# microsoft/Spartan2

Measured on AMD Instinct MI355X. Metric: sha256_spartan prove(): R1CS constraints/sec (prove wall-clock in ms_per_step), higher is better.
Workload: dtype u256 modular integer (8 x u32 Montgomery limbs; T256 scalar/base fields)

## Files before the change

spartan2_amd/csrc/capi_sparse.hip:

```cpp
#include <algorithm>
#include <cstring>
#include <string>
#include <vector>

#include "core.hpp"
#include "device_utils.hpp"
#include "kernels_sat.hpp"

using sp::fail;
typedef FqP S;

namespace spk {

struct SplitDev {
  const unsigned* sptr;
  const unsigned* sidx;
  const signed char* scode;
  const unsigned* gptr;
  const unsigned* gidx;
  const fe_t* gval;
};

__device__ __forceinline__ fe_t small_mul(int code, const fe_t& x) {
  const int a = code < 0 ? -code : code;
  fe_t r;
  switch (a) {
    case 1: r = x; break;
    case 2: r = fe_dbl<S>(x); break;
    case 3: r = fe_add<S>(fe_dbl<S>(x), x); break;
    case 4: r = fe_dbl<S>(fe_dbl<S>(x)); break;
// ... 77 lines not shown
    while (pending) {
      const int owner = __ffsll((long long)pending) - 1;
      pending &= pending - 1;
      const size_t r = wbase + (size_t)owner;
      const fe_t part = wave_sum(gather_major(m, r, z, lane, 64));
      if ((int)lane == owner) acc = part;
    }
    if (valid) {
      if (base) acc = fe_add<S>(acc, base[row]);
      out[row] = acc;
    }
  }
}

__global__ void __launch_bounds__(256) k_round0_products(const fe_t* __restrict__ A, const fe_t* __restrict__ B, const fe_t* __restrict__ C, size_t half,
                                                         fe_t* __restrict__ p0, fe_t* __restrict__ p1) {
  for (size_t i = (size_t)blockIdx.x * blockDim.x + threadIdx.x; i < half; i += (size_t)gridDim.x * blockDim.x) {
    const fe_t a0 = A[i], a1 = A[i + half], b0 = B[i], b1 = B[i + half], c0 = C[i];
    p0[i] = fe_sub<S>(fe_mul<S>(a0, b0), c0);
    p1[i] = fe_mul<S>(fe_sub<S>(a1, a0), fe_sub<S>(b1, b0));
  }
}

struct PolyAbcArgs {
  SplitDev m[3];
  fe_t r, r2;
};
constexpr unsigned LONG_COLUMN = 512;
__device__ __forceinline__ unsigned col_len(const PolyAbcArgs& a, size_t col) {
  unsigned n = 0;
#pragma unroll
  for (int i = 0; i < 3; ++i) n += (a.m[i].sptr[col + 1] - a.m[i].sptr[col]) + (a.m[i].gptr[col + 1] - a.m[i].gptr[col]);
  return n;
}
constexpr unsigned LONG_NB_MAX = 128;
__device__ __forceinline__ unsigned long_nb(unsigned len) {
  unsigned nb = (len + 2047) / 2048;
  return nb < 1 ? 1 : (nb > LONG_NB_MAX ? LONG_NB_MAX : nb);
}
__global__ void __launch_bounds__(256) k_polyabc_short_and_long(PolyAbcArgs a, const fe_t* __restrict__ rx, const unsigned* __restrict__ order, size_t n_short,
                                                                fe_t* __restrict__ out, const unsigned* __restrict__ long_cols, unsigned n_long,
                                                                fe_t* __restrict__ partials, unsigned* __restrict__ tickets, unsigned short_blocks,
                                                                size_t zero_from, size_t zero_n, int permuted) {
  __shared__ fe_t smem[3 * 4];
  __shared__ unsigned s_last;
  const unsigned long_blocks = LONG_NB_MAX * n_long;
  if (blockIdx.x >= long_blocks + short_blocks) {
    uint4* z = reinterpret_cast<uint4*>(out + zero_from);
    const size_t n16 = zero_n * 2, nb = gridDim.x - long_blocks - short_blocks;
    for (size_t i = (size_t)(blockIdx.x - long_blocks - short_blocks) * blockDim.x + threadIdx.x; i < n16; i += nb * blockDim.x) z[i] = make_uint4(0u, 0u, 0u, 0u);
    return;
  }
  if (blockIdx.x < long_blocks) {
    const unsigned by = blockIdx.x / LONG_NB_MAX, bx = blockIdx.x % LONG_NB_MAX;
    const size_t col = long_cols[by];
    const size_t at = permuted ? n_short + by : col;
    const unsigned nb = long_nb(col_len(a, at));
    if (bx >= nb) return;
    fe_t acc[3];
#pragma unroll
    for (int i = 0; i < 3; ++i) acc[i] = gather_major(a.m[i], at, rx, bx * blockDim.x + threadIdx.x, nb * blockDim.x);
    block_sum<3>(acc, smem);
    fe_t* trip = partials + ((size_t)by * LONG_NB_MAX) * 3;
    if (threadIdx.x == 0) {
      unsigned* dst = reinterpret_cast<unsigned*>(trip + (size_t)bx * 3);
#pragma unroll
      for (int i = 0; i < 3; ++i)
#pragma unroll
        for (int w = 0; w < 8; ++w) __hip_atomic_store(dst + 8 * i + w, acc[i].v[w], __ATOMIC_RELAXED, __HIP_MEMORY_SCOPE_AGENT);
      s_last = __hip_atomic_fetch_add(tickets + by, 1u, __ATOMIC_ACQ_REL, __HIP_MEMORY_SCOPE_AGENT) == nb - 1 ? 1u : 0u;
    }
    __syncthreads();
    if (!s_last) return;
#pragma unroll
    for (int i = 0; i < 3; ++i) {
      acc[i] = fe_zero();
      if (threadIdx.x < nb) {
        const unsigned* src = reinterpret_cast<const unsigned*>(trip + (size_t)threadIdx.x * 3 + i);
#pragma unroll
        for (int w = 0; w < 8; ++w) acc[i].v[w] = __hip_atomic_load(src + w, __ATOMIC_RELAXED, __HIP_MEMORY_SCOPE_AGENT);
      }
    }
    __syncthreads();
    block_sum<3>(acc, smem);
    if (threadIdx.x == 0) {
      __hip_atomic_store(tickets + by, 0u, __ATOMIC_RELAXED, __HIP_MEMORY_SCOPE_AGENT);
      out[col] = fe_add<S>(fe_add<S>(acc[0], fe_mul<S>(a.r, acc[1])), fe_mul<S>(a.r2, acc[2]));
    }
    return;
  }
  const size_t nblk = short_blocks;
  for (size_t i = (size_t)(blockIdx.x - long_blocks) * blockDim.x + threadIdx.x; i < n_short; i += nblk * blockDim.x) {
    const size_t col = order[i], at = permuted ? i : col;
    fe_t sa = gather_major_x4(a.m[0], at, rx), sb = gather_major_x4(a.m[1], at, rx), sc = gather_major_x4(a.m[2], at, rx);
    if (!fe_is_zero(sb)) sa = fe_add<S>(sa, fe_mul<S>(a.r, sb));
    if (!fe_is_zero(sc)) sa = fe_add<S>(sa, fe_mul<S>(a.r2, sc));
    out[col] = sa;
  }
}
}

#include "kernels_mateval.hpp"
#include "kernels_polyabc_batch.hpp"
#include "kernels_spmv_multi.hpp"
#include "kernels_nifs_layers.hpp"

namespace {

struct SplitHost {
  std::vector<unsigned> sptr, sidx, gptr, gidx;
  std::vector<signed char> scode;
  std::vector<fe_t> gval;
};
struct SplitOnDevice {
  unsigned *sptr = nullptr, *sidx = nullptr, *gptr = nullptr, *gidx = nullptr;
  signed char* scode = nullptr;
  fe_t* gval = nullptr;
  unsigned max_len = 0;
  spk::SplitDev view() const { return spk::SplitDev{sptr, sidx, scode, gptr, gidx, gval}; }
  void release() {
// ... 25 lines not shown

template <class T>
int upload(T** dst, const std::vector<T>& src) {
  size_t bytes = (src.empty() ? 1 : src.size()) * sizeof(T);
  hipError_t e = hipMalloc((void**)dst, bytes);
  if (e != hipSuccess) return fail(SP_ERR_NO_DEVICE, std::string("hipMalloc: ") + hipGetErrorString(e));
  if (!src.empty()) e = hipMemcpy(*dst, src.data(), src.size() * sizeof(T), hipMemcpyHostToDevice);
  if (e != hipSuccess) return fail(SP_ERR_NO_DEVICE, std::string("hipMemcpy: ") + hipGetErrorString(e));
  return SP_OK;
}
int upload_split(const SplitHost& h, SplitOnDevice* d) {
  int rc;
  if ((rc = upload(&d->sptr, h.sptr))) return rc;
  if ((rc = upload(&d->sidx, h.sidx))) return rc;
  if ((rc = upload(&d->scode, h.scode))) return rc;
  if ((rc = upload(&d->gptr, h.gptr))) return rc;
  if ((rc = upload(&d->gidx, h.gidx))) return rc;
  d->max_len = 0;
  for (size_t i = 0; i + 1 < h.sptr.size(); ++i) {
    const unsigned l = (h.sptr[i + 1] - h.sptr[i]) + (h.gptr[i + 1] - h.gptr[i]);
    if (l > d->max_len) d->max_len = l;
  }
  return upload(&d->gval, h.gval);
}

struct Entry {
  unsigned major, minor;
  int code;
  fe_t val;
};
SplitHost build_split(size_t n_major, const std::vector<Entry>& es) {
  SplitHost h;
  h.sptr.assign(n_major + 1, 0);
  h.gptr.assign(n_major + 1, 0);
  for (const Entry& e : es) (e.code ? h.sptr : h.gptr)[e.major + 1]++;
  for (size_t i = 0; i < n_major; ++i) {
    h.sptr[i + 1] += h.sptr[i];
    h.gptr[i + 1] += h.gptr[i];
  }
  h.sidx.resize(h.sptr[n_major]);
  h.scode.resize(h.sptr[n_major]);
  h.gidx.resize(h.gptr[n_major]);
  h.gval.resize(h.gptr[n_major]);
  std::vector<unsigned> sc(h.sptr.begin(), h.sptr.end() - 1), gc(h.gptr.begin(), h.gptr.end() - 1);
  for (const Entry& e : es) {
    if (e.code) {
      unsigned p = sc[e.major]++;
      h.sidx[p] = e.minor;
      h.scode[p] = (signed char)e.code;
    } else {
      unsigned p = gc[e.major]++;
      h.gidx[p] = e.minor;
      h.gval[p] = e.val;
    }
  }
  return h;
}

}

struct sp_shape {
  sp_dims dims;
  size_t num_vars = 0, num_cols = 0;
  SplitOnDevice row[3];
  SplitOnDevice filtered[3];
  SplitOnDevice col[3];
  unsigned* d_long_cols = nullptr;
  unsigned* d_short_order = nullptr;
  size_t n_short = 0;
  size_t n_long_cols = 0;
  bool col_permuted = false;
  uint64_t nnz[3] = {0, 0, 0}, nnz_filtered[3] = {0, 0, 0};
};

extern "C" {

int sp_shape_from_csr(sp_ctx* c, const sp_csr* A, const sp_csr* Bm, const sp_csr* C, const sp_dims* dims, sp_shape** out) {
  (void)c;
  sp_shape* s = new sp_shape();
  s->dims = *dims;
  s->num_vars = dims->num_shared + dims->num_precommitted + dims->num_rest;
  s->num_cols = s->num_vars + 1 + dims->num_public + dims->num_challenges;
  const size_t nrows = dims->num_cons, col_min = dims->num_shared + dims->num_precommitted, nr_used = dims->num_cons_unpadded;
  const sp_csr* M[3] = {A, Bm, C};
  Classifier cls;
  std::vector<unsigned> col_count(s->num_cols, 0);
  std::vector<SplitHost> col_host(3);
  for (int m = 0; m < 3; ++m) {
    const size_t nnz = M[m]->indptr[nrows];
    s->nnz[m] = nnz;
    std::vector<Entry> all, filt, bycol;
    all.reserve(nnz);
    for (size_t r = 0; r < nrows; ++r) {
      for (uint64_t k = M[m]->indptr[r]; k < M[m]->indptr[r + 1]; ++k) {
        Entry e;
        e.major = (unsigned)r;
        e.minor = M[m]->indices[k];
        if (e.minor >= s->num_cols) {
          delete s;
          return fail(SP_ERR_INVALID_INPUT_LENGTH, "sp_shape_from_csr: column index out of range");
        }
        memcpy(&e.val, M[m]->data + 4 * k, 32);
        e.code = cls.code(e.val);
        all.push_back(e);
        if (r < nr_used && e.minor >= col_min) filt.push_back(e);
      }
    }
    s->nnz_filtered[m] = filt.size();
    std::vector<unsigned> cptr(s->num_cols + 1, 0);
    for (const Entry& e : all)
      if (e.major < nr_used) cptr[e.minor + 1]++;
    for (size_t i = 0; i < s->num_cols; ++i) cptr[i + 1] += cptr[i];
    bycol.resize(cptr[s->num_cols]);
    {
      std::vector<unsigned> cur(cptr.begin(), cptr.end() - 1);
      for (const Entry& e : all)
        if (e.major < nr_used) {
          Entry t = e;
          t.major = e.minor;
          t.minor = e.major;
          bycol[cur[e.minor]++] = t;
        }
    }
    for (size_t i = 0; i < s->num_cols; ++i) col_count[i] += cptr[i + 1] - cptr[i];
    int rc;
    col_host[m] = build_split(s->num_cols, bycol);
    if ((rc = upload_split(build_split(nrows, all), &s->row[m])) || (rc = upload_split(build_split(nrows, filt), &s->filtered[m]))) {
      delete s;
      return rc;
    }
  }
  std::vector<unsigned> long_cols;
  for (size_t i = 0; i < s->num_cols; ++i)
    if (col_count[i] >= spk::LONG_COLUMN) long_cols.push_back((unsigned)i);
  s->n_long_cols = long_cols.size();
  int rc = upload(&s->d_long_cols, long_cols);
  if (rc) {
    sp_shape_free(s);
    return rc;
  }
  {
    std::vector<unsigned> order;
    order.reserve(s->num_cols);
    for (size_t i = 0; i < s->num_cols; ++i)
      if (col_count[i] < spk::LONG_COLUMN) order.push_back((unsigned)i);
    auto cnt6 = [&](unsigned col, unsigned out6[6]) {
      for (int m = 0; m < 3; ++m) {
        out6[2 * m] = col_host[m].sptr[col + 1] - col_host[m].sptr[col];
        out6[2 * m + 1] = col_host[m].gptr[col + 1] - col_host[m].gptr[col];
      }
    };
    auto by_len = [&](unsigned x, unsigned y) {
      if (col_count[x] != col_count[y]) return col_count[x] > col_count[y];
      unsigned a[6], b[6];
      cnt6(x, a);
      cnt6(y, b);
      for (int k = 0; k < 5; ++k)
        if (a[k] != b[k]) return a[k] > b[k];
      return false;
    };
    static const int order_mode = [] {
      const char* e = getenv("SPARTAN_POLYABC_ORDER");
      return !e ? 0 : (e[0] == 'n' ? 1 : (e[0] == 'w' ? 2 : 0));
    }();
    if (order_mode == 0) std::stable_sort(order.begin(), order.end(), by_len);
    else if (order_mode == 2)
    {
      const char* w = getenv("SPARTAN_POLYABC_WINDOW");
      const size_t win = w && atol(w) > 0 ? (size_t)atol(w) : 4096;
      for (size_t lo = 0; lo < order.size(); lo += win) std::stable_sort(order.begin() + lo, order.begin() + std::min(order.size(), lo + win), by_len);
    }
    s->n_short = order.size();
    if ((rc = upload(&s->d_short_order, order))) {
      sp_shape_free(s);
      return rc;
    }
    static const bool permuted = [] {
      const char* e = getenv("SPARTAN_POLYABC_LAYOUT");
      return !(e && e[0] == 'n');
    }();
    s->col_permuted = permuted;
    std::vector<unsigned> seq;
    if (permuted) {
      seq = order;
      seq.insert(seq.end(), long_cols.begin(), long_cols.end());
    }
    for (int m = 0; m < 3; ++m) {
      if (!permuted) {
        if ((rc = upload_split(col_host[m], &s->col[m]))) {
          sp_shape_free(s);
          return rc;
        }
        continue;
      }
      const SplitHost& h = col_host[m];
      SplitHost q;
      q.sptr.assign(seq.size() + 1, 0);
      q.gptr.assign(seq.size() + 1, 0);
      q.sidx.reserve(h.sidx.size());
      q.scode.reserve(h.scode.size());
      q.gidx.reserve(h.gidx.size());
      q.gval.reserve(h.gval.size());
      for (size_t pos = 0; pos < seq.size(); ++pos) {
        const unsigned col = seq[pos];
        q.sidx.insert(q.sidx.end(), h.sidx.begin() + h.sptr[col], h.sidx.begin() + h.sptr[col + 1]);
        q.scode.insert(q.scode.end(), h.scode.begin() + h.sptr[col], h.scode.begin() + h.sptr[col + 1]);
        q.gidx.insert(q.gidx.end(), h.gidx.begin() + h.gptr[col], h.gidx.begin() + h.gptr[col + 1]);
        q.gval.insert(q.gval.end(), h.gval.begin() + h.gptr[col], h.gval.begin() + h.gptr[col + 1]);
        q.sptr[pos + 1] = (unsigned)q.sidx.size();
        q.gptr[pos + 1] = (unsigned)q.gidx.size();
      }
      if ((rc = upload_split(q, &s->col[m]))) {
        sp_shape_free(s);
        return rc;
      }
    }
  }
  SP_HIP(hipDeviceSynchronize());
  *out = s;
  return SP_OK;
}
void sp_shape_free(sp_shape* s) {
  if (!s) return;
  for (int m = 0; m < 3; ++m) {
    s->row[m].release();
    s->filtered[m].release();
    s->col[m].release();
  }
  hipFree(s->d_long_cols);
  hipFree(s->d_short_order);
  delete s;
}

int sp_shape_info(const sp_shape* s, uint64_t out[8]) {
  if (!s || !out) return fail(SP_ERR_INVALID_INPUT_LENGTH, "sp_shape_info: null argument");
  for (int m = 0; m < 3; ++m) {
    out[m] = s->nnz[m];
    out[3 + m] = s->nnz_filtered[m];
  }
  out[6] = s->n_long_cols;
  out[7] = s->n_short;
  return SP_OK;
}

static int spmv3(sp_ctx* c, const sp_shape* s, const SplitOnDevice* mats, const uint64_t* nnz, const sp_table* z, const sp_table* const* base,
                 sp_table** outs, const char* what) {
  const size_t nrows = s->dims.num_cons;
  if (z->len != s->num_cols) return fail(SP_ERR_INVALID_WITNESS_LENGTH, "multiply_vec: z has the wrong length");
  spk::Spmv3Args a;
  for (int m = 0; m < 3; ++m) {
    if (outs[m]->cap < nrows) return fail(SP_ERR_INVALID_INPUT_LENGTH, "multiply_vec: output table too short");
// ... 68 lines not shown
  const sp_table* base[3] = {caz, cbz, ccz};
  return spmv3(c, s, s->filtered, s->nnz_filtered, z, base, outs, "spmv_incremental");
}

int sp_multiply_vec_incremental_round0(sp_ctx* c, const sp_shape* s, const sp_table* z, const sp_table* caz, const sp_table* cbz, const sp_table* ccz, sp_table* az,
                                       sp_table* bz, sp_table* cz, sp_table* p0, sp_table* p1) {
  const size_t nrows = s->dims.num_cons, half = nrows / 2;
  if (nrows < 2) return fail(SP_ERR_INVALID_INPUT_LENGTH, "multiply_vec_incremental_round0: needs at least two rows");
  if (p0->cap < half || p1->cap < half) return fail(SP_ERR_INVALID_INPUT_LENGTH, "multiply_vec_incremental_round0: product tables too short");
  int rc = sp_multiply_vec_incremental(c, s, z, caz, cbz, ccz, az, bz, cz);
  if (rc) return rc;
  p0->len = p1->len = half;
  p0->lo_eff = p0->hi_eff = p1->lo_eff = p1->hi_eff = (size_t)-1;
  size_t blocks = (half + 255) / 256;
  if (blocks > 8192) blocks = 8192;
  c->timed("round0_products", 224ull * half, [&] { hipLaunchKernelGGL(spk::k_round0_products, dim3((unsigned)blocks), dim3(256), 0, c->stream, az->d, bz->d, cz->d, half, p0->d, p1->d); });
  return SP_OK;
}

int sp_poly_abc(sp_ctx* c, const sp_shape* s, const sp_table* rx, const uint64_t r_[4], size_t out_len, sp_table* out) {
  if (rx->len != s->dims.num_cons) return fail(SP_ERR_INVALID_INPUT_LENGTH, "poly_ABC: rx must have num_cons elements");
  if (out_len < s->num_cols || out->cap < out_len) return fail(SP_ERR_INVALID_INPUT_LENGTH, "poly_ABC: output too short");
  spk::PolyAbcArgs a;
  for (int m = 0; m < 3; ++m) a.m[m] = s->col[m].view();
  memcpy(&a.r, r_, 32);
  a.r2 = fe_mul<S>(a.r, a.r);
  const size_t ticket_bytes = (s->n_long_cols + 1) * sizeof(unsigned);
  const bool fresh = c->ws_bytes[sp_ctx::WS_POLYABC_TICKETS] < ticket_bytes;
  fe_t* partials = (fe_t*)c->workspace(sp_ctx::WS_POLYABC_PARTIALS, (s->n_long_cols + 1) * spk::LONG_NB_MAX * 3 * sizeof(fe_t));
  unsigned* tickets = (unsigned*)c->workspace(sp_ctx::WS_POLYABC_TICKETS, ticket_bytes);
  if (!partials || !tickets) return SP_ERR_NO_DEVICE;
  if (fresh) SP_HIP(hipMemsetAsync(tickets, 0, c->ws_bytes[sp_ctx::WS_POLYABC_TICKETS], c->stream));
  size_t blocks = (s->n_short + 255) / 256;
  if (blocks > 4096) blocks = 4096;
  if (blocks == 0) blocks = 1;
  const uint64_t bytes = 36ull * (s->nnz[0] + s->nnz[1] + s->nnz[2]) + 32ull * out_len;
  const size_t zero_n = out_len - s->num_cols;
  size_t zblocks = (2 * zero_n + 256 * 16 - 1) / (256 * 16);
  if (zblocks > 2048) zblocks = 2048;
  c->timed("poly_abc", bytes, [&] {
    hipLaunchKernelGGL(spk::k_polyabc_short_and_long, dim3((unsigned)(blocks + spk::LONG_NB_MAX * s->n_long_cols + zblocks)), dim3(256), 0, c->stream, a, rx->d, s->d_short_order,
                       s->n_short, out->d, s->d_long_cols, (unsigned)s->n_long_cols, partials, tickets, (unsigned)blocks, (size_t)s->num_cols, zero_n, s->col_permuted ? 1 : 0);
  });
  return SP_OK;
}

size_t sp_poly_abc_batch_chunk(void) { return (size_t)spk::PAB_KC; }
// ... 16 lines not shown
  const size_t ticket_bytes = (s->n_long_cols + 1) * sizeof(unsigned);
  const bool fresh = c->ws_bytes[sp_ctx::WS_POLYABC_BATCH_TICKETS] < ticket_bytes;
  unsigned* tickets = (unsigned*)c->workspace(sp_ctx::WS_POLYABC_BATCH_TICKETS, ticket_bytes);
  if (!tickets) return SP_ERR_NO_DEVICE;
  if (fresh) SP_HIP(hipMemsetAsync(tickets, 0, c->ws_bytes[sp_ctx::WS_POLYABC_BATCH_TICKETS], c->stream));
  fe_t* partials = (fe_t*)c->workspace(sp_ctx::WS_POLYABC_BATCH_PARTIALS, (s->n_long_cols + 1) * spk::LONG_NB_MAX * 3 * KC * sizeof(fe_t));
  fe_t* pyr = (fe_t*)c->workspace(sp_ctx::WS_POLYABC_BATCH_PYRAMIDS, KC * pyr_stride * sizeof(fe_t));
  fe_t* E = (fe_t*)c->workspace(sp_ctx::WS_POLYABC_BATCH_EQ, KC * nrows * sizeof(fe_t));
  if (!partials || !pyr || !E) return SP_ERR_NO_DEVICE;
  size_t blocks = (s->n_short + 255) / 256;
  if (blocks > 4096) blocks = 4096;
  if (blocks == 0) blocks = 1;
  const size_t zero_n = out_len - s->num_cols;
  size_t zblocks = (2 * zero_n + 256 * 16 - 1) / (256 * 16);
  if (zblocks > 2048) zblocks = 2048;
  size_t eblocks = (KC * nrows + 255) / 256;
  if (eblocks > 8192) eblocks = 8192;
  const uint64_t nnz = s->nnz[0] + s->nnz[1] + s->nnz[2];
  const dim3 grid((unsigned)(blocks + spk::LONG_NB_MAX * s->n_long_cols + zblocks));
  for (size_t k0 = 0; k0 < count; k0 += KC) {
    const size_t kc = std::min<size_t>(KC, count - k0);
    spk::PabPoints pts;
    spk::PabArgs a;
    for (int m = 0; m < 3; ++m) a.m[m] = s->col[m].view();
    for (size_t j = 0; j < KC; ++j) {
      const size_t k = k0 + (j < kc ? j : 0);
      if (ell) memcpy(pts.v[j], r_x + 4 * ell * k, ell * sizeof(fe_t));
      memcpy(&a.r[j], r_ + 4 * k, sizeof(fe_t));
      a.r2[j] = fe_mul<S>(a.r[j], a.r[j]);
      a.out[j] = out[k]->d;
    }
    a.kc = (int)kc;
    c->timed_kernel("eq_levels_batch", (uint64_t)kc * pyr_stride * sizeof(fe_t), spk::k_pab_eq_levels, dim3(2, (unsigned)kc), dim3(1024), pts, (int)ell, hi_bits, pyr,
                    (unsigned long long)pyr_stride, (unsigned long long)pyr_hi);
    c->timed_kernel("eq_table_batch", 32ull * nrows * kc, spk::k_pab_eq_outer, dim3((unsigned)eblocks), dim3(256), (const fe_t*)pyr, (unsigned long long)pyr_stride,
                    (unsigned long long)spk::eq_level_offset(hi_bits), (unsigned long long)(pyr_hi + spk::eq_level_offset(lo_bits)), lo_bits, nrows, (int)kc, E);
    const uint64_t bytes = 5ull * nnz + 24ull * s->num_cols + kc * (32ull * nnz + 32ull * out_len);
    if (kc == KC)
      c->timed_kernel("poly_abc_batch", bytes, spk::k_pab_walk<true>, grid, dim3(256), a, (const fe_t*)E, (const unsigned*)s->d_short_order, s->n_short,
                      (const unsigned*)s->d_long_cols, (unsigned)s->n_long_cols, partials, tickets, (unsigned)blocks, (size_t)s->num_cols, zero_n, s->col_permuted ? 1 : 0);
    else
      c->timed_kernel("poly_abc_batch", bytes, spk::k_pab_walk<false>, grid, dim3(256), a, (const fe_t*)E, (const unsigned*)s->d_short_order, s->n_short,
                      (const unsigned*)s->d_long_cols, (unsigned)s->n_long_cols, partials, tickets, (unsigned)blocks, (size_t)s->num_cols, zero_n, s->col_permuted ? 1 : 0);
  }
  return SP_OK;
}

// ... 164 lines not shown
```

spartan2_amd/csrc/kernels_polyabc_batch.hpp:

```cpp
#pragma once
#include "kernels_shared.hpp"

#ifndef POLYABC_BATCH_KC
#define POLYABC_BATCH_KC 4
#endif

namespace spk {

constexpr int PAB_KC = POLYABC_BATCH_KC;
static_assert(PAB_KC == 2 || PAB_KC == 4, "the in-flight depth of pab_gather_col is written for 2 and 4");
constexpr int PAB_MAX_ELL = 28;
constexpr int PAB_INFLIGHT = 4 / PAB_KC;

struct PabPoints {
  fe_t v[PAB_KC][PAB_MAX_ELL];
};
__global__ void __launch_bounds__(1024) k_pab_eq_levels(PabPoints p, int ell, int hi_bits, fe_t* __restrict__ pyr, unsigned long long stride, unsigned long long pyr_hi) {
  __shared__ fe_t lv[EQ_LDS_ENTRIES];
  const int j = blockIdx.y;
  fe_t* o = pyr + (size_t)j * stride;
  if (blockIdx.x == 0) eq_levels_block(&p.v[j][hi_bits - 1], hi_bits, o, lv);
  else eq_levels_block(&p.v[j][ell - 1], ell - hi_bits, o + pyr_hi, lv);
}

__global__ void __launch_bounds__(256) k_pab_eq_outer(const fe_t* __restrict__ pyr, unsigned long long stride, unsigned long long off_hi, unsigned long long off_lo, int lo_bits,
                                                      size_t n_rows, int kc, fe_t* __restrict__ E) {
  const size_t mask = ((size_t)1 << lo_bits) - 1, total = n_rows * PAB_KC;
  for (size_t t = (size_t)blockIdx.x * blockDim.x + threadIdx.x; t < total; t += (size_t)gridDim.x * blockDim.x) {
    const size_t row = t / PAB_KC;
    const int j = (int)(t % PAB_KC);
    if (j >= kc) continue;
    const fe_t* __restrict__ q = pyr + (size_t)j * stride;
    E[t] = fe_mul<S>(q[off_hi + (row >> lo_bits)], q[off_lo + (row & mask)]);
  }
}

struct PabArgs {
  SplitDev m[3];
  fe_t r[PAB_KC], r2[PAB_KC];
  fe_t* out[PAB_KC];
  int kc;
};

template <bool FULL>
__device__ __forceinline__ void pab_gather_strided(const SplitDev& m, size_t major, const fe_t* __restrict__ E, int kc, unsigned first, unsigned step, fe_t (&acc)[PAB_KC]) {
  for (unsigned k = m.sptr[major] + first, e = m.sptr[major + 1]; k < e; k += step) {
    const fe_t* __restrict__ x = E + (size_t)m.sidx[k] * PAB_KC;
    const int code = m.scode[k];
#pragma unroll
    for (int j = 0; j < PAB_KC; ++j)
      if (FULL || j < kc) acc[j] = acc_small(acc[j], code, x[j]);
  }
  for (unsigned k = m.gptr[major] + first, e = m.gptr[major + 1]; k < e; k += step) {
    const fe_t* __restrict__ x = E + (size_t)m.gidx[k] * PAB_KC;
    const fe_t v = m.gval[k];
#pragma unroll
    for (int j = 0; j < PAB_KC; ++j)
      if (FULL || j < kc) acc[j] = fe_add<S>(acc[j], fe_mul<S>(v, x[j]));
  }
}
template <bool FULL>
__device__ __forceinline__ void pab_gather_col(const SplitDev& m, size_t major, const fe_t* __restrict__ E, int kc, fe_t (&acc)[PAB_KC]) {
  unsigned k = m.sptr[major];
  const unsigned e = m.sptr[major + 1];
  for (; k + PAB_INFLIGHT <= e; k += PAB_INFLIGHT) {
    unsigned idx[PAB_INFLIGHT];
    int code[PAB_INFLIGHT];
#pragma unroll
    for (int u = 0; u < PAB_INFLIGHT; ++u) {
      idx[u] = m.sidx[k + u];
      code[u] = m.scode[k + u];
    }
    fe_t x[PAB_INFLIGHT][PAB_KC];
#pragma unroll
    for (int u = 0; u < PAB_INFLIGHT; ++u)
#pragma unroll
      for (int j = 0; j < PAB_KC; ++j)
        if (FULL || j < kc) x[u][j] = E[(size_t)idx[u] * PAB_KC + j];
#pragma unroll
    for (int u = 0; u < PAB_INFLIGHT; ++u)
#pragma unroll
      for (int j = 0; j < PAB_KC; ++j)
        if (FULL || j < kc) acc[j] = acc_small(acc[j], code[u], x[u][j]);
  }
  for (; k < e; ++k) {
    const fe_t* __restrict__ x = E + (size_t)m.sidx[k] * PAB_KC;
    const int code = m.scode[k];
#pragma unroll
    for (int j = 0; j < PAB_KC; ++j)
      if (FULL || j < kc) acc[j] = acc_small(acc[j], code, x[j]);
  }
  for (unsigned g = m.gptr[major], ge = m.gptr[major + 1]; g < ge; ++g) {
    const fe_t* __restrict__ x = E + (size_t)m.gidx[g] * PAB_KC;
    const fe_t v = m.gval[g];
#pragma unroll
    for (int j = 0; j < PAB_KC; ++j)
      if (FULL || j < kc) acc[j] = fe_add<S>(acc[j], fe_mul<S>(v, x[j]));
  }
}
__device__ __forceinline__ unsigned pab_col_len(const PabArgs& a, size_t col) {
  unsigned n = 0;
#pragma unroll
  for (int i = 0; i < 3; ++i) n += (a.m[i].sptr[col + 1] - a.m[i].sptr[col]) + (a.m[i].gptr[col + 1] - a.m[i].gptr[col]);
  return n;
}

template <bool FULL>
__global__ void __launch_bounds__(256) k_pab_walk(PabArgs a, const fe_t* __restrict__ E, const unsigned* __restrict__ order, size_t n_short,
                                                  const unsigned* __restrict__ long_cols, unsigned n_long, fe_t* __restrict__ partials, unsigned* __restrict__ tickets,
                                                  unsigned short_blocks, size_t zero_from, size_t zero_n, int permuted) {
  __shared__ fe_t smem[PAB_KC * 4];
  __shared__ unsigned s_last;
  const int kc = FULL ? PAB_KC : a.kc;
  const unsigned long_blocks = LONG_NB_MAX * n_long;
  if (blockIdx.x >= long_blocks + short_blocks) {
    const size_t n16 = zero_n * 2, nb = gridDim.x - long_blocks - short_blocks;
#pragma unroll
    for (int j = 0; j < PAB_KC; ++j) {
      if (!FULL && j >= kc) break;
      uint4* z = reinterpret_cast<uint4*>(a.out[j] + zero_from);
      for (size_t i = (size_t)(blockIdx.x - long_blocks - short_blocks) * blockDim.x + threadIdx.x; i < n16; i += nb * blockDim.x) z[i] = make_uint4(0u, 0u, 0u, 0u);
    }
    return;
  }
  fe_t acc[PAB_KC], tot[PAB_KC];
  if (blockIdx.x < long_blocks) {
    const unsigned by = blockIdx.x / LONG_NB_MAX, bx = blockIdx.x % LONG_NB_MAX;
    const size_t col = long_cols[by];
    const size_t at = permuted ? n_short + by : col;
    const unsigned nb = long_nb(pab_col_len(a, at));
    if (bx >= nb) return;
    fe_t* trip = partials + (size_t)by * LONG_NB_MAX * 3 * PAB_KC;
#pragma unroll 1
    for (int i = 0; i < 3; ++i) {
#pragma unroll
      for (int j = 0; j < PAB_KC; ++j) acc[j] = fe_zero();
      pab_gather_strided<FULL>(a.m[i], at, E, kc, bx * blockDim.x + threadIdx.x, nb * blockDim.x, acc);
      if (i) __syncthreads();
      block_sum<PAB_KC>(acc, smem);
      if (threadIdx.x == 0) {
        unsigned* dst = reinterpret_cast<unsigned*>(trip + ((size_t)bx * 3 + i) * PAB_KC);
#pragma unroll
        for (int j = 0; j < PAB_KC; ++j)
#pragma unroll
          for (int w = 0; w < 8; ++w) __hip_atomic_store(dst + 8 * j + w, acc[j].v[w], __ATOMIC_RELAXED, __HIP_MEMORY_SCOPE_AGENT);
      }
    }
    if (threadIdx.x == 0) s_last = __hip_atomic_fetch_add(tickets + by, 1u, __ATOMIC_ACQ_REL, __HIP_MEMORY_SCOPE_AGENT) == nb - 1 ? 1u : 0u;
    __syncthreads();
    if (!s_last) return;
#pragma unroll 1
    for (int i = 0; i < 3; ++i) {
#pragma unroll
      for (int j = 0; j < PAB_KC; ++j) acc[j] = fe_zero();
      if (threadIdx.x < nb) {
        const unsigned* src = reinterpret_cast<const unsigned*>(trip + ((size_t)threadIdx.x * 3 + i) * PAB_KC);
#pragma unroll
        for (int j = 0; j < PAB_KC; ++j)
#pragma unroll
          for (int w = 0; w < 8; ++w) acc[j].v[w] = __hip_atomic_load(src + 8 * j + w, __ATOMIC_RELAXED, __HIP_MEMORY_SCOPE_AGENT);
      }
      __syncthreads();
      block_sum<PAB_KC>(acc, smem);
      if (threadIdx.x == 0) {
#pragma unroll
        for (int j = 0; j < PAB_KC; ++j) tot[j] = i == 0 ? acc[j] : fe_add<S>(tot[j], fe_mul<S>(i == 1 ? a.r[j] : a.r2[j], acc[j]));
      }
    }
    if (threadIdx.x == 0) {
      __hip_atomic_store(tickets + by, 0u, __ATOMIC_RELAXED, __HIP_MEMORY_SCOPE_AGENT);
#pragma unroll
      for (int j = 0; j < PAB_KC; ++j)
        if (FULL || j < kc) a.out[j][col] = tot[j];
    }
    return;
  }
  const size_t nblk = short_blocks;
  for (size_t i = (size_t)(blockIdx.x - long_blocks) * blockDim.x + threadIdx.x; i < n_short; i += nblk * blockDim.x) {
    const size_t col = order[i], at = permuted ? i : col;
#pragma unroll
    for (int j = 0; j < PAB_KC; ++j) tot[j] = fe_zero();
    pab_gather_col<FULL>(a.m[0], at, E, kc, tot);
#pragma unroll
    for (int j = 0; j < PAB_KC; ++j) acc[j] = fe_zero();
    pab_gather_col<FULL>(a.m[1], at, E, kc, acc);
#pragma unroll
    for (int j = 0; j < PAB_KC; ++j)
      if (!fe_is_zero(acc[j])) tot[j] = fe_add<S>(tot[j], fe_mul<S>(a.r[j], acc[j]));
#pragma unroll
    for (int j = 0; j < PAB_KC; ++j) acc[j] = fe_zero();
    pab_gather_col<FULL>(a.m[2], at, E, kc, acc);
#pragma unroll
    for (int j = 0; j < PAB_KC; ++j)
      if (!fe_is_zero(acc[j])) tot[j] = fe_add<S>(tot[j], fe_mul<S>(a.r2[j], acc[j]));
#pragma unroll
    for (int j = 0; j < PAB_KC; ++j)
      if (FULL || j < kc) a.out[j][col] = tot[j];
  }
}

}
```

Baseline: 1.022 billion.

## Merge A/B/C column-major matrices into one row-keyed stream with value dictionary

Replaces the three separate split (small-code plus general-value) column-major layouts used by poly_ABC with one merged stream. Each entry holds a row and the A, B and C codes together, and general coefficients become indices into a deduplicated value dictionary, with a residual list for overflow. The single-proof kernel stages the dictionary in LDS when it fits. The aim is to read each rx/E row once per column instead of up to three times and to shrink index and value traffic. The cost is 12-byte entries that carry zero codes for absent matrices and extra host build time. The batched kernel still walks the merged stream once per matrix.

```diff
diff --git a/spartan2_amd/csrc/capi_sparse.hip b/spartan2_amd/csrc/capi_sparse.hip
--- a/spartan2_amd/csrc/capi_sparse.hip
+++ b/spartan2_amd/csrc/capi_sparse.hip
@@ -1,4 +1,5 @@
 #include <algorithm>
+#include <array>
 #include <cstring>
 #include <string>
 #include <vector>
@@ -6,6 +7,7 @@
 #include "core.hpp"
 #include "device_utils.hpp"
 #include "kernels_sat.hpp"
+#include "polyabc_merged.hpp"
 
 using sp::fail;
 typedef FqP S;
@@ -129,27 +131,93 @@
   }
 }
 
+struct MergedDev {
+  const unsigned* ptr;
+  const unsigned* ent;
+  const fe_t* dict;
+  unsigned n_dict;
+  int has_residual;
+  const unsigned* rptr;
+  const unsigned* rrow;
+  const unsigned char* rmat;
+  const fe_t* rval;
+};
+struct MEnt {
+  unsigned row, ab, c;
+};
+__device__ __forceinline__ MEnt merged_entry(const MergedDev& m, unsigned k) { return reinterpret_cast<const MEnt*>(m.ent)[k]; }
+constexpr unsigned CODE_DICT0 = pabm::CODE_DICT0;
+__device__ __forceinline__ int small_of(unsigned code) { return code <= 7 ? (int)code : 7 - (int)code; }
+__device__ __forceinline__ void acc_code(fe_t& acc, unsigned code, const fe_t& x, const fe_t* __restrict__ dict) {
+  if (code == 0) return;
+  if (code < CODE_DICT0) acc = acc_small(acc, small_of(code), x);
+  else acc = fe_add<S>(acc, fe_mul<S>(dict[code - CODE_DICT0], x));
+}
+__device__ __forceinline__ void acc_entry(fe_t (&s)[3], const MEnt& t, const fe_t& x, const fe_t* __restrict__ dict) {
+  acc_code(s[0], t.ab & 0xffffu, x, dict);
+  acc_code(s[1], t.ab >> 16, x, dict);
+  acc_code(s[2], t.c, x, dict);
+}
+__device__ __forceinline__ void acc_residual(fe_t (&s)[3], const MergedDev& m, unsigned g, const fe_t* __restrict__ x) {
+  const fe_t v = fe_mul<S>(m.rval[g], x[m.rrow[g]]);
+  const unsigned which = m.rmat[g];
+  if (which == 0) s[0] = fe_add<S>(s[0], v);
+  else if (which == 1) s[1] = fe_add<S>(s[1], v);
+  else s[2] = fe_add<S>(s[2], v);
+}
+__device__ __forceinline__ void merged_col_x4(const MergedDev& m, size_t at, const fe_t* __restrict__ x, const fe_t* __restrict__ dict, fe_t (&s)[3]) {
+  const unsigned e = m.ptr[at + 1];
+  for (unsigned k = m.ptr[at]; k < e; k += 4) {
+    MEnt t[4];
+#pragma unroll
+    for (unsigned u = 0; u < 4; ++u) {
+      t[u] = MEnt{0u, 0u, 0u};
+      if (k + u < e) t[u] = merged_entry(m, k + u);
+    }
+    fe_t v[4];
+#pragma unroll
+    for (unsigned u = 0; u < 4; ++u) {
+      v[u] = fe_zero();
+      if (k + u < e) v[u] = x[t[u].row];
+    }
+    acc_entry(s, t[0], v[0], dict);
+    acc_entry(s, t[1], v[1], dict);
+    acc_entry(s, t[2], v[2], dict);
+    acc_entry(s, t[3], v[3], dict);
+  }
+  if (m.has_residual)
+    for (unsigned g = m.rptr[at], ge = m.rptr[at + 1]; g < ge; ++g) acc_residual(s, m, g, x);
+}
+__device__ __forceinline__ void merged_col_strided(const MergedDev& m, size_t at, const fe_t* __restrict__ x, const fe_t* __restrict__ dict, unsigned first, unsigned step,
+                                                   fe_t (&s)[3]) {
+  for (unsigned k = m.ptr[at] + first, e = m.ptr[at + 1]; k < e; k += step) {
+    const MEnt t = merged_entry(m, k);
+    acc_entry(s, t, x[t.row], dict);
+  }
+  if (m.has_residual)
+    for (unsigned g = m.rptr[at] + first, ge = m.rptr[at + 1]; g < ge; g += step) acc_residual(s, m, g, x);
+}
+
 struct PolyAbcArgs {
-  SplitDev m[3];
+  MergedDev m;
   fe_t r, r2;
 };
 constexpr unsigned LONG_COLUMN = 512;
-__device__ __forceinline__ unsigned col_len(const PolyAbcArgs& a, size_t col) {
-  unsigned n = 0;
-#pragma unroll
-  for (int i = 0; i < 3; ++i) n += (a.m[i].sptr[col + 1] - a.m[i].sptr[col]) + (a.m[i].gptr[col + 1] - a.m[i].gptr[col]);
-  return n;
-}
 constexpr unsigned LONG_NB_MAX = 128;
 __device__ __forceinline__ unsigned long_nb(unsigned len) {
   unsigned nb = (len + 2047) / 2048;
   return nb < 1 ? 1 : (nb > LONG_NB_MAX ? LONG_NB_MAX : nb);
 }
+#ifndef POLYABC_LDS_DICT
+#define POLYABC_LDS_DICT 256
+#endif
+constexpr unsigned LDS_DICT_MAX = POLYABC_LDS_DICT;
 __global__ void __launch_bounds__(256) k_polyabc_short_and_long(PolyAbcArgs a, const fe_t* __restrict__ rx, const unsigned* __restrict__ order, size_t n_short,
                                                                 fe_t* __restrict__ out, const unsigned* __restrict__ long_cols, unsigned n_long,
                                                                 fe_t* __restrict__ partials, unsigned* __restrict__ tickets, unsigned short_blocks,
                                                                 size_t zero_from, size_t zero_n, int permuted) {
   __shared__ fe_t smem[3 * 4];
+  __shared__ fe_t sdict[LDS_DICT_MAX ? LDS_DICT_MAX : 1];
   __shared__ unsigned s_last;
   const unsigned long_blocks = LONG_NB_MAX * n_long;
   if (blockIdx.x >= long_blocks + short_blocks) {
@@ -158,15 +226,15 @@
     for (size_t i = (size_t)(blockIdx.x - long_blocks - short_blocks) * blockDim.x + threadIdx.x; i < n16; i += nb * blockDim.x) z[i] = make_uint4(0u, 0u, 0u, 0u);
     return;
   }
+  const bool lds_dict = LDS_DICT_MAX && a.m.n_dict <= LDS_DICT_MAX;
   if (blockIdx.x < long_blocks) {
     const unsigned by = blockIdx.x / LONG_NB_MAX, bx = blockIdx.x % LONG_NB_MAX;
     const size_t col = long_cols[by];
     const size_t at = permuted ? n_short + by : col;
-    const unsigned nb = long_nb(col_len(a, at));
+    const unsigned nb = long_nb(a.m.ptr[at + 1] - a.m.ptr[at]);
     if (bx >= nb) return;
-    fe_t acc[3];
-#pragma unroll
-    for (int i = 0; i < 3; ++i) acc[i] = gather_major(a.m[i], at, rx, bx * blockDim.x + threadIdx.x, nb * blockDim.x);
+    fe_t acc[3] = {fe_zero(), fe_zero(), fe_zero()};
+    merged_col_strided(a.m, at, rx, a.m.dict, bx * blockDim.x + threadIdx.x, nb * blockDim.x, acc);
     block_sum<3>(acc, smem);
     fe_t* trip = partials + ((size_t)by * LONG_NB_MAX) * 3;
     if (threadIdx.x == 0) {
@@ -196,13 +264,19 @@
     }
     return;
   }
+  if (lds_dict) {
+    for (unsigned i = threadIdx.x; i < a.m.n_dict; i += blockDim.x) sdict[i] = a.m.dict[i];
+    __syncthreads();
+  }
   const size_t nblk = short_blocks;
   for (size_t i = (size_t)(blockIdx.x - long_blocks) * blockDim.x + threadIdx.x; i < n_short; i += nblk * blockDim.x) {
     const size_t col = order[i], at = permuted ? i : col;
-    fe_t sa = gather_major_x4(a.m[0], at, rx), sb = gather_major_x4(a.m[1], at, rx), sc = gather_major_x4(a.m[2], at, rx);
-    if (!fe_is_zero(sb)) sa = fe_add<S>(sa, fe_mul<S>(a.r, sb));
-    if (!fe_is_zero(sc)) sa = fe_add<S>(sa, fe_mul<S>(a.r2, sc));
-    out[col] = sa;
+    fe_t s[3] = {fe_zero(), fe_zero(), fe_zero()};
+    if (lds_dict) merged_col_x4(a.m, at, rx, sdict, s);
+    else merged_col_x4(a.m, at, rx, a.m.dict, s);
+    if (!fe_is_zero(s[1])) s[0] = fe_add<S>(s[0], fe_mul<S>(a.r, s[1]));
+    if (!fe_is_zero(s[2])) s[0] = fe_add<S>(s[0], fe_mul<S>(a.r2, s[2]));
+    out[col] = s[0];
   }
 }
 }
@@ -274,6 +348,34 @@
     if (l > d->max_len) d->max_len = l;
   }
   return upload(&d->gval, h.gval);
+}
+
+struct MergedOnDevice {
+  unsigned *ptr = nullptr, *ent = nullptr, *rptr = nullptr, *rrow = nullptr;
+  unsigned char* rmat = nullptr;
+  fe_t *dict = nullptr, *rval = nullptr;
+  unsigned n_dict = 0;
+  bool has_residual = false;
+  spk::MergedDev view() const { return spk::MergedDev{ptr, ent, dict, n_dict, has_residual ? 1 : 0, rptr, rrow, rmat, rval}; }
+  void release() {
+    hipFree(ptr);
+    hipFree(ent);
+    hipFree(rptr);
+    hipFree(rrow);
+    hipFree(rmat);
+    hipFree(dict);
+    hipFree(rval);
+  }
+};
+static_assert(sizeof(pabm::Val) == sizeof(fe_t), "a dictionary value is a field element as stored");
+int upload_merged(const pabm::Merged& h, MergedOnDevice* d) {
+  int rc;
+  if ((rc = upload(&d->ptr, h.ptr)) || (rc = upload(&d->ent, h.ent)) || (rc = upload(reinterpret_cast<pabm::Val**>(&d->dict), h.dict))) return rc;
+  d->n_dict = (unsigned)h.dict.size();
+  d->has_residual = h.has_residual;
+  if (!h.has_residual) return SP_OK;
+  if ((rc = upload(&d->rptr, h.rptr)) || (rc = upload(&d->rrow, h.rrow)) || (rc = upload(&d->rmat, h.rmat))) return rc;
+  return upload(reinterpret_cast<pabm::Val**>(&d->rval), h.rval);
 }
 
 struct Entry {
@@ -316,7 +418,7 @@
   size_t num_vars = 0, num_cols = 0;
   SplitOnDevice row[3];
   SplitOnDevice filtered[3];
-  SplitOnDevice col[3];
+  MergedOnDevice col;
   unsigned* d_long_cols = nullptr;
   unsigned* d_short_order = nullptr;
   size_t n_short = 0;
@@ -337,11 +439,12 @@
   const sp_csr* M[3] = {A, Bm, C};
   Classifier cls;
   std::vector<unsigned> col_count(s->num_cols, 0);
-  std::vector<SplitHost> col_host(3);
+  pabm::ColMajor col_host[3];
+  pabm::Values general;
   for (int m = 0; m < 3; ++m) {
     const size_t nnz = M[m]->indptr[nrows];
     s->nnz[m] = nnz;
-    std::vector<Entry> all, filt, bycol;
+    std::vector<Entry> all, filt;
     all.reserve(nnz);
     for (size_t r = 0; r < nrows; ++r) {
       for (uint64_t k = M[m]->indptr[r]; k < M[m]->indptr[r + 1]; ++k) {
@@ -359,24 +462,29 @@
       }
     }
     s->nnz_filtered[m] = filt.size();
-    std::vector<unsigned> cptr(s->num_cols + 1, 0);
+    std::vector<unsigned>& cptr = col_host[m].ptr;
+    cptr.assign(s->num_cols + 1, 0);
     for (const Entry& e : all)
       if (e.major < nr_used) cptr[e.minor + 1]++;
     for (size_t i = 0; i < s->num_cols; ++i) cptr[i + 1] += cptr[i];
-    bycol.resize(cptr[s->num_cols]);
+    col_host[m].ent.resize(cptr[s->num_cols]);
     {
       std::vector<unsigned> cur(cptr.begin(), cptr.end() - 1);
       for (const Entry& e : all)
         if (e.major < nr_used) {
-          Entry t = e;
-          t.major = e.minor;
-          t.minor = e.major;
-          bycol[cur[e.minor]++] = t;
+          pabm::Item t;
+          t.row = e.major;
+          if (e.code) t.code = e.code;
+          else {
+            pabm::Val v;
+            memcpy(&v, &e.val, sizeof v);
+            t.code = pabm::GENERAL0 + (int32_t)general.id(v);
+          }
+          col_host[m].ent[cur[e.minor]++] = t;
         }
     }
     for (size_t i = 0; i < s->num_cols; ++i) col_count[i] += cptr[i + 1] - cptr[i];
     int rc;
-    col_host[m] = build_split(s->num_cols, bycol);
     if ((rc = upload_split(build_split(nrows, all), &s->row[m])) || (rc = upload_split(build_split(nrows, filt), &s->filtered[m]))) {
       delete s;
       return rc;
@@ -396,21 +504,14 @@
     order.reserve(s->num_cols);
     for (size_t i = 0; i < s->num_cols; ++i)
       if (col_count[i] < spk::LONG_COLUMN) order.push_back((unsigned)i);
-    auto cnt6 = [&](unsigned col, unsigned out6[6]) {
-      for (int m = 0; m < 3; ++m) {
-        out6[2 * m] = col_host[m].sptr[col + 1] - col_host[m].sptr[col];
-        out6[2 * m + 1] = col_host[m].gptr[col + 1] - col_host[m].gptr[col];
-      }
-    };
-    auto by_len = [&](unsigned x, unsigned y) {
-      if (col_count[x] != col_count[y]) return col_count[x] > col_count[y];
-      unsigned a[6], b[6];
-      cnt6(x, a);
-      cnt6(y, b);
-      for (int k = 0; k < 5; ++k)
-        if (a[k] != b[k]) return a[k] > b[k];
-      return false;
-    };
+    std::vector<std::array<unsigned, 4>> key(s->num_cols);
+    for (unsigned col : order) {
+      unsigned general_n = 0;
+      for (int m = 0; m < 3; ++m)
+        for (unsigned k = col_host[m].ptr[col]; k < col_host[m].ptr[col + 1]; ++k) general_n += col_host[m].ent[k].code >= pabm::GENERAL0;
+      key[col] = {pabm::merged_len(col_host, col), general_n, col_host[0].ptr[col + 1] - col_host[0].ptr[col], col_host[1].ptr[col + 1] - col_host[1].ptr[col]};
+    }
+    auto by_len = [&](unsigned x, unsigned y) { return key[x] > key[y]; };
     static const int order_mode = [] {
       const char* e = getenv("SPARTAN_POLYABC_ORDER");
       return !e ? 0 : (e[0] == 'n' ? 1 : (e[0] == 'w' ? 2 : 0));
@@ -436,36 +537,13 @@
     if (permuted) {
       seq = order;
       seq.insert(seq.end(), long_cols.begin(), long_cols.end());
-    }
-    for (int m = 0; m < 3; ++m) {
-      if (!permuted) {
-        if ((rc = upload_split(col_host[m], &s->col[m]))) {
-          sp_shape_free(s);
-          return rc;
-        }
-        continue;
-      }
-      const SplitHost& h = col_host[m];
-      SplitHost q;
-      q.sptr.assign(seq.size() + 1, 0);
-      q.gptr.assign(seq.size() + 1, 0);
-      q.sidx.reserve(h.sidx.size());
-      q.scode.reserve(h.scode.size());
-      q.gidx.reserve(h.gidx.size());
-      q.gval.reserve(h.gval.size());
-      for (size_t pos = 0; pos < seq.size(); ++pos) {
-        const unsigned col = seq[pos];
-        q.sidx.insert(q.sidx.end(), h.sidx.begin() + h.sptr[col], h.sidx.begin() + h.sptr[col + 1]);
-        q.scode.insert(q.scode.end(), h.scode.begin() + h.sptr[col], h.scode.begin() + h.sptr[col + 1]);
-        q.gidx.insert(q.gidx.end(), h.gidx.begin() + h.gptr[col], h.gidx.begin() + h.gptr[col + 1]);
-        q.gval.insert(q.gval.end(), h.gval.begin() + h.gptr[col], h.gval.begin() + h.gptr[col + 1]);
-        q.sptr[pos + 1] = (unsigned)q.sidx.size();
-        q.gptr[pos + 1] = (unsigned)q.gidx.size();
-      }
-      if ((rc = upload_split(q, &s->col[m]))) {
-        sp_shape_free(s);
-        return rc;
-      }
+    } else {
+      seq.resize(s->num_cols);
+      for (size_t i = 0; i < s->num_cols; ++i) seq[i] = (unsigned)i;
+    }
+    if ((rc = upload_merged(pabm::build(col_host, general, seq), &s->col))) {
+      sp_shape_free(s);
+      return rc;
     }
   }
   SP_HIP(hipDeviceSynchronize());
@@ -477,8 +555,8 @@
   for (int m = 0; m < 3; ++m) {
     s->row[m].release();
     s->filtered[m].release();
-    s->col[m].release();
-  }
+  }
+  s->col.release();
   hipFree(s->d_long_cols);
   hipFree(s->d_short_order);
   delete s;
@@ -593,7 +671,7 @@
   if (rx->len != s->dims.num_cons) return fail(SP_ERR_INVALID_INPUT_LENGTH, "poly_ABC: rx must have num_cons elements");
   if (out_len < s->num_cols || out->cap < out_len) return fail(SP_ERR_INVALID_INPUT_LENGTH, "poly_ABC: output too short");
   spk::PolyAbcArgs a;
-  for (int m = 0; m < 3; ++m) a.m[m] = s->col[m].view();
+  a.m = s->col.view();
   memcpy(&a.r, r_, 32);
   a.r2 = fe_mul<S>(a.r, a.r);
   const size_t ticket_bytes = (s->n_long_cols + 1) * sizeof(unsigned);
@@ -656,7 +734,7 @@
     const size_t kc = std::min<size_t>(KC, count - k0);
     spk::PabPoints pts;
     spk::PabArgs a;
-    for (int m = 0; m < 3; ++m) a.m[m] = s->col[m].view();
+    a.m = s->col.view();
     for (size_t j = 0; j < KC; ++j) {
       const size_t k = k0 + (j < kc ? j : 0);
       if (ell) memcpy(pts.v[j], r_x + 4 * ell * k, ell * sizeof(fe_t));
diff --git a/spartan2_amd/csrc/kernels_polyabc_batch.hpp b/spartan2_amd/csrc/kernels_polyabc_batch.hpp
--- a/spartan2_amd/csrc/kernels_polyabc_batch.hpp
+++ b/spartan2_amd/csrc/kernels_polyabc_batch.hpp
@@ -8,9 +8,8 @@
 namespace spk {
 
 constexpr int PAB_KC = POLYABC_BATCH_KC;
-static_assert(PAB_KC == 2 || PAB_KC == 4, "the in-flight depth of pab_gather_col is written for 2 and 4");
+static_assert(PAB_KC == 2 || PAB_KC == 4, "the interleaved eq tables and the walk are measured for 2 and 4 proofs a chunk");
 constexpr int PAB_MAX_ELL = 28;
-constexpr int PAB_INFLIGHT = 4 / PAB_KC;
 
 struct PabPoints {
   fe_t v[PAB_KC][PAB_MAX_ELL];
@@ -36,73 +35,72 @@
 }
 
 struct PabArgs {
-  SplitDev m[3];
+  MergedDev m;
   fe_t r[PAB_KC], r2[PAB_KC];
   fe_t* out[PAB_KC];
   int kc;
 };
 
 template <bool FULL>
-__device__ __forceinline__ void pab_gather_strided(const SplitDev& m, size_t major, const fe_t* __restrict__ E, int kc, unsigned first, unsigned step, fe_t (&acc)[PAB_KC]) {
-  for (unsigned k = m.sptr[major] + first, e = m.sptr[major + 1]; k < e; k += step) {
-    const fe_t* __restrict__ x = E + (size_t)m.sidx[k] * PAB_KC;
-    const int code = m.scode[k];
-#pragma unroll
-    for (int j = 0; j < PAB_KC; ++j)
-      if (FULL || j < kc) acc[j] = acc_small(acc[j], code, x[j]);
-  }
-  for (unsigned k = m.gptr[major] + first, e = m.gptr[major + 1]; k < e; k += step) {
-    const fe_t* __restrict__ x = E + (size_t)m.gidx[k] * PAB_KC;
-    const fe_t v = m.gval[k];
+__device__ __forceinline__ void pab_acc_code(fe_t (&acc)[PAB_KC], unsigned code, const fe_t (&x)[PAB_KC], int kc, const fe_t* __restrict__ dict) {
+  if (code == 0) return;
+  if (code < CODE_DICT0) {
+    const int c = small_of(code);
+#pragma unroll
+    for (int j = 0; j < PAB_KC; ++j)
+      if (FULL || j < kc) acc[j] = acc_small(acc[j], c, x[j]);
+  } else {
+    const fe_t v = dict[code - CODE_DICT0];
 #pragma unroll
     for (int j = 0; j < PAB_KC; ++j)
       if (FULL || j < kc) acc[j] = fe_add<S>(acc[j], fe_mul<S>(v, x[j]));
   }
 }
-template <bool FULL>
-__device__ __forceinline__ void pab_gather_col(const SplitDev& m, size_t major, const fe_t* __restrict__ E, int kc, fe_t (&acc)[PAB_KC]) {
-  unsigned k = m.sptr[major];
-  const unsigned e = m.sptr[major + 1];
-  for (; k + PAB_INFLIGHT <= e; k += PAB_INFLIGHT) {
-    unsigned idx[PAB_INFLIGHT];
-    int code[PAB_INFLIGHT];
-#pragma unroll
-    for (int u = 0; u < PAB_INFLIGHT; ++u) {
-      idx[u] = m.sidx[k + u];
-      code[u] = m.scode[k + u];
-    }
-    fe_t x[PAB_INFLIGHT][PAB_KC];
-#pragma unroll
-    for (int u = 0; u < PAB_INFLIGHT; ++u)
-#pragma unroll
-      for (int j = 0; j < PAB_KC; ++j)
-        if (FULL || j < kc) x[u][j] = E[(size_t)idx[u] * PAB_KC + j];
-#pragma unroll
-    for (int u = 0; u < PAB_INFLIGHT; ++u)
-#pragma unroll
-      for (int j = 0; j < PAB_KC; ++j)
-        if (FULL || j < kc) acc[j] = acc_small(acc[j], code[u], x[u][j]);
-  }
-  for (; k < e; ++k) {
-    const fe_t* __restrict__ x = E + (size_t)m.sidx[k] * PAB_KC;
-    const int code = m.scode[k];
-#pragma unroll
-    for (int j = 0; j < PAB_KC; ++j)
-      if (FULL || j < kc) acc[j] = acc_small(acc[j], code, x[j]);
-  }
-  for (unsigned g = m.gptr[major], ge = m.gptr[major + 1]; g < ge; ++g) {
-    const fe_t* __restrict__ x = E + (size_t)m.gidx[g] * PAB_KC;
-    const fe_t v = m.gval[g];
-#pragma unroll
-    for (int j = 0; j < PAB_KC; ++j)
-      if (FULL || j < kc) acc[j] = fe_add<S>(acc[j], fe_mul<S>(v, x[j]));
-  }
-}
-__device__ __forceinline__ unsigned pab_col_len(const PabArgs& a, size_t col) {
-  unsigned n = 0;
-#pragma unroll
-  for (int i = 0; i < 3; ++i) n += (a.m[i].sptr[col + 1] - a.m[i].sptr[col]) + (a.m[i].gptr[col + 1] - a.m[i].gptr[col]);
-  return n;
+__device__ __forceinline__ unsigned pab_code_of(const MEnt& t, int which) { return which == 0 ? t.ab & 0xffffu : (which == 1 ? t.ab >> 16 : t.c); }
+template <bool FULL>
+__device__ __forceinline__ void pab_acc_residual(fe_t (&acc)[PAB_KC], const MergedDev& m, unsigned g, int which, const fe_t* __restrict__ E, int kc) {
+  if ((int)m.rmat[g] != which) return;
+  const fe_t* __restrict__ x = E + (size_t)m.rrow[g] * PAB_KC;
+  const fe_t v = m.rval[g];
+#pragma unroll
+  for (int j = 0; j < PAB_KC; ++j)
+    if (FULL || j < kc) acc[j] = fe_add<S>(acc[j], fe_mul<S>(v, x[j]));
+}
+template <bool FULL>
+__device__ __forceinline__ void pab_acc_entry(fe_t (&acc)[PAB_KC], unsigned code, unsigned row, const fe_t* __restrict__ E, int kc, const fe_t* __restrict__ dict) {
+  if (code == 0) return;
+  fe_t x[PAB_KC];
+#pragma unroll
+  for (int j = 0; j < PAB_KC; ++j)
+    if (FULL || j < kc) x[j] = E[(size_t)row * PAB_KC + j];
+  pab_acc_code<FULL>(acc, code, x, kc, dict);
+}
+template <bool FULL>
+__device__ __forceinline__ void pab_gather_strided(const MergedDev& m, size_t at, int which, const fe_t* __restrict__ E, int kc, unsigned first, unsigned step, fe_t (&acc)[PAB_KC]) {
+  for (unsigned k = m.ptr[at] + first, e = m.ptr[at + 1]; k < e; k += step) {
+    const MEnt t = merged_entry(m, k);
+    pab_acc_entry<FULL>(acc, pab_code_of(t, which), t.row, E, kc, m.dict);
+  }
+  if (m.has_residual)
+    for (unsigned g = m.rptr[at] + first, ge = m.rptr[at + 1]; g < ge; g += step) pab_acc_residual<FULL>(acc, m, g, which, E, kc);
+}
+template <bool FULL>
+__device__ __forceinline__ void pab_gather_col(const MergedDev& m, size_t at, int which, const fe_t* __restrict__ E, int kc, fe_t (&acc)[PAB_KC]) {
+  const unsigned e = m.ptr[at + 1];
+  for (unsigned k = m.ptr[at]; k < e; k += 4) {
+    MEnt t[4];
+#pragma unroll
+    for (unsigned u = 0; u < 4; ++u) {
+      t[u] = MEnt{0u, 0u, 0u};
+      if (k + u < e) t[u] = merged_entry(m, k + u);
+    }
+    pab_acc_entry<FULL>(acc, pab_code_of(t[0], which), t[0].row, E, kc, m.dict);
+    pab_acc_entry<FULL>(acc, pab_code_of(t[1], which), t[1].row, E, kc, m.dict);
+    pab_acc_entry<FULL>(acc, pab_code_of(t[2], which), t[2].row, E, kc, m.dict);
+    pab_acc_entry<FULL>(acc, pab_code_of(t[3], which), t[3].row, E, kc, m.dict);
+  }
+  if (m.has_residual)
+    for (unsigned g = m.rptr[at], ge = m.rptr[at + 1]; g < ge; ++g) pab_acc_residual<FULL>(acc, m, g, which, E, kc);
 }
 
 template <bool FULL>
@@ -128,14 +126,14 @@
     const unsigned by = blockIdx.x / LONG_NB_MAX, bx = blockIdx.x % LONG_NB_MAX;
     const size_t col = long_cols[by];
     const size_t at = permuted ? n_short + by : col;
-    const unsigned nb = long_nb(pab_col_len(a, at));
+    const unsigned nb = long_nb(a.m.ptr[at + 1] - a.m.ptr[at]);
     if (bx >= nb) return;
     fe_t* trip = partials + (size_t)by * LONG_NB_MAX * 3 * PAB_KC;
 #pragma unroll 1
     for (int i = 0; i < 3; ++i) {
 #pragma unroll
       for (int j = 0; j < PAB_KC; ++j) acc[j] = fe_zero();
-      pab_gather_strided<FULL>(a.m[i], at, E, kc, bx * blockDim.x + threadIdx.x, nb * blockDim.x, acc);
+      pab_gather_strided<FULL>(a.m, at, i, E, kc, bx * blockDim.x + threadIdx.x, nb * blockDim.x, acc);
       if (i) __syncthreads();
       block_sum<PAB_KC>(acc, smem);
       if (threadIdx.x == 0) {
@@ -180,16 +178,16 @@
     const size_t col = order[i], at = permuted ? i : col;
 #pragma unroll
     for (int j = 0; j < PAB_KC; ++j) tot[j] = fe_zero();
-    pab_gather_col<FULL>(a.m[0], at, E, kc, tot);
+    pab_gather_col<FULL>(a.m, at, 0, E, kc, tot);
 #pragma unroll
     for (int j = 0; j < PAB_KC; ++j) acc[j] = fe_zero();
-    pab_gather_col<FULL>(a.m[1], at, E, kc, acc);
+    pab_gather_col<FULL>(a.m, at, 1, E, kc, acc);
 #pragma unroll
     for (int j = 0; j < PAB_KC; ++j)
       if (!fe_is_zero(acc[j])) tot[j] = fe_add<S>(tot[j], fe_mul<S>(a.r[j], acc[j]));
 #pragma unroll
     for (int j = 0; j < PAB_KC; ++j) acc[j] = fe_zero();
-    pab_gather_col<FULL>(a.m[2], at, E, kc, acc);
+    pab_gather_col<FULL>(a.m, at, 2, E, kc, acc);
 #pragma unroll
     for (int j = 0; j < PAB_KC; ++j)
       if (!fe_is_zero(acc[j])) tot[j] = fe_add<S>(tot[j], fe_mul<S>(a.r2[j], acc[j]));
diff --git a/spartan2_amd/csrc/polyabc_merged.hpp b/spartan2_amd/csrc/polyabc_merged.hpp
--- /dev/null
+++ b/spartan2_amd/csrc/polyabc_merged.hpp
@@ -0,0 +1,151 @@
+#pragma once
+#include <stdint.h>
+#include <string.h>
+
+#include <algorithm>
+#include <unordered_map>
+#include <vector>
+
+namespace pabm {
+
+struct Val {
+  uint32_t w[8];
+  bool operator==(const Val& o) const { return memcmp(w, o.w, sizeof w) == 0; }
+};
+struct ValHash {
+  size_t operator()(const Val& v) const {
+    uint64_t h = 0x9e3779b97f4a7c15ull;
+    for (int i = 0; i < 8; ++i) h = (h ^ v.w[i]) * 0x100000001b3ull;
+    return (size_t)(h ^ (h >> 29));
+  }
+};
+
+struct Values {
+  std::unordered_map<Val, uint32_t, ValHash> index;
+  std::vector<Val> distinct;
+  std::vector<uint32_t> count;
+  uint32_t id(const Val& v) {
+    auto r = index.emplace(v, (uint32_t)distinct.size());
+    if (r.second) {
+      distinct.push_back(v);
+      count.push_back(0);
+    }
+    ++count[r.first->second];
+    return r.first->second;
+  }
+};
+constexpr int32_t GENERAL0 = 8;
+struct Item {
+  uint32_t row;
+  int32_t code;
+};
+struct ColMajor {
+  std::vector<uint32_t> ptr;
+  std::vector<Item> ent;
+};
+
+constexpr uint32_t CODE_DICT0 = 15;
+constexpr size_t DICT_MAX = 65536 - CODE_DICT0;
+
+struct Merged {
+  std::vector<uint32_t> ptr;
+  std::vector<uint32_t> ent;
+  std::vector<Val> dict;
+  bool has_residual = false;
+  std::vector<uint32_t> rptr;
+  std::vector<uint32_t> rrow;
+  std::vector<uint8_t> rmat;
+  std::vector<Val> rval;
+};
+
+inline uint32_t small_code(int code) { return code > 0 ? (uint32_t)code : (uint32_t)(7 - code); }
+inline int small_from_code(uint32_t code) { return code <= 7 ? (int)code : 7 - (int)code; }
+
+inline uint32_t merged_len(const ColMajor m[3], size_t col) {
+  uint32_t k[3], e[3], n = 0;
+  for (int i = 0; i < 3; ++i) {
+    k[i] = m[i].ptr[col];
+    e[i] = m[i].ptr[col + 1];
+  }
+  for (;;) {
+    bool any = false;
+    uint32_t row = 0;
+    for (int i = 0; i < 3; ++i)
+      if (k[i] < e[i] && (!any || m[i].ent[k[i]].row < row)) {
+        row = m[i].ent[k[i]].row;
+        any = true;
+      }
+    if (!any) return n;
+    uint32_t mult = 0;
+    for (int i = 0; i < 3; ++i) {
+      uint32_t c = 0;
+      while (k[i] < e[i] && m[i].ent[k[i]].row == row) ++k[i], ++c;
+      mult = std::max(mult, c);
+    }
+    n += mult;
+  }
+}
+
+inline Merged build(const ColMajor m[3], const Values& values, const std::vector<uint32_t>& seq, size_t dict_max = DICT_MAX) {
+  Merged out;
+  const std::vector<Val>& distinct = values.distinct;
+  std::vector<uint32_t> by_count(distinct.size());
+  for (size_t i = 0; i < by_count.size(); ++i) by_count[i] = (uint32_t)i;
+  if (distinct.size() > dict_max) {
+    std::stable_sort(by_count.begin(), by_count.end(), [&](uint32_t a, uint32_t b) { return values.count[a] > values.count[b]; });
+    out.has_residual = true;
+  }
+  std::vector<uint32_t> code_of(distinct.size(), 0);
+  const size_t n_dict = std::min(distinct.size(), dict_max);
+  out.dict.resize(n_dict);
+  for (size_t i = 0; i < n_dict; ++i) {
+    out.dict[i] = distinct[by_count[i]];
+    code_of[by_count[i]] = CODE_DICT0 + (uint32_t)i;
+  }
+  out.ptr.assign(seq.size() + 1, 0);
+  if (out.has_residual) out.rptr.assign(seq.size() + 1, 0);
+  for (size_t pos = 0; pos < seq.size(); ++pos) {
+    const size_t col = seq[pos];
+    uint32_t k[3], e[3];
+    for (int i = 0; i < 3; ++i) {
+      k[i] = m[i].ptr[col];
+      e[i] = m[i].ptr[col + 1];
+    }
+    for (;;) {
+      bool any = false;
+      uint32_t row = 0;
+      for (int i = 0; i < 3; ++i)
+        if (k[i] < e[i] && (!any || m[i].ent[k[i]].row < row)) {
+          row = m[i].ent[k[i]].row;
+          any = true;
+        }
+      if (!any) break;
+      for (;;) {
+        uint32_t code[3] = {0, 0, 0};
+        bool took = false, coded = false;
+        for (int i = 0; i < 3; ++i) {
+          if (k[i] >= e[i] || m[i].ent[k[i]].row != row) continue;
+          const Item& it = m[i].ent[k[i]++];
+          took = true;
+          code[i] = it.code < GENERAL0 ? small_code(it.code) : code_of[it.code - GENERAL0];
+          if (code[i]) coded = true;
+          else {
+            out.rrow.push_back(row);
+            out.rmat.push_back((uint8_t)i);
+            out.rval.push_back(distinct[it.code - GENERAL0]);
+          }
+        }
+        if (!took) break;
+        if (!coded) continue;
+        out.ent.push_back(row);
+        out.ent.push_back(code[0] | code[1] << 16);
+        out.ent.push_back(code[2]);
+      }
+    }
+    out.ptr[pos + 1] = (uint32_t)(out.ent.size() / 3);
+    if (out.has_residual) out.rptr[pos + 1] = (uint32_t)out.rrow.size();
+  }
+  return out;
+}
+
+}
```

Measured after the change: 1.035 billion, median of 4. About the same (+1.3%).
